# piwell/CS348B-pbrt

Hardware: AMD Instinct MI355X
Metric: volumetric photon-gather throughput (camera samples through PhotonVolumeIntegrator::Li per second) (higher is better)
Workload: dtype f32

## Files before the change

cs348b-pbrt_amd/csrc/pvol_api.hip:

```cpp
#include <hip/hip_runtime.h>
#include <math.h>
#include <stdlib.h>
#include <string.h>
#include <algorithm>
#include <mutex>
#include <new>
#include <vector>

#include "pvol_dev.h"

#include "pvol_host.h"

static bool ok(hipError_t e) { return e == hipSuccess; }

extern "C" {

int pvol_abi_version(void) { return PVOL_ABI_VERSION; }

const char *pvol_strerror(int s) {
    switch (s) {
    case PVOL_OK: return "ok";
    case PVOL_E_INVALID: return "invalid argument";
    case PVOL_E_NO_DEVICE: return "no usable HIP device (this library has no CPU path)";
    case PVOL_E_NO_SCENE: return "no scene set";
// ... 12 lines not shown
}

void pvol_default_params(pvol_params *p) {
    memset(p, 0, sizeof(*p));
    p->step_size = 1.f;
    p->n_used = 250;
    p->max_dist = 0.1f;
    p->n_volume_photons = 0;
    p->shooter_step_size = 0.1f;
    p->max_photon_depth = 5;
    p->n_caustic_photons = 20000;
    p->n_indirect_photons = 10000;
    p->final_gather = 1;
    p->device = 0;
    p->grid_cell_scale = 0.f;
    p->keep_surface_photons = 0;
}

int pvol_create(const pvol_params *params, pvol_ctx **out) {
    if (!params || !out) return PVOL_E_INVALID;
    *out = 0;
    if (params->n_used < 1 || !(params->step_size > 0.f) || !(params->max_dist > 0.f)) return PVOL_E_INVALID;
    if (params->n_used > 576) return PVOL_E_UNSUPPORTED;
    int n = 0;
    if (!ok(hipGetDeviceCount(&n)) || n <= 0 || params->device < 0 || params->device >= n) return PVOL_E_NO_DEVICE;
    if (!ok(hipSetDevice(params->device))) return PVOL_E_NO_DEVICE;
    pvol_ctx *c = new (std::nothrow) pvol_ctx();
    if (!c) return PVOL_E_NO_MEMORY;
    c->params = *params;
    { const char *fs = getenv("PVOL_FORCE_SEQ"); c->forceSeq = fs && fs[0] == '1'; }
    { const char *ng = getenv("PVOL_NO_GROUP"); c->noGroup = ng && ng[0] == '1'; }
    { const char *nl = getenv("PVOL_NO_LITE"); c->noLite = nl && nl[0] == '1'; }
    { const char *nm = getenv("PVOL_NO_MOMENTS"); c->noMoments = nm && nm[0] == '1'; }
    { const char *tg = getenv("PVOL_TILE_GENERAL"); c->tileGeneral = tg && tg[0] == '1'; }
    { const char *gw = getenv("PVOL_GROUP_WAVES"); if (gw) c->groupWavesPerCU = std::max(1, atoi(gw)); }
    { const char *tw = getenv("PVOL_TILE_WAVES"); if (tw) c->tileWaves = std::max(0, atoi(tw)); }
    { const char *fw = getenv("PVOL_FIX_WAVES"); if (fw) c->fixWavesPerCU = std::max(1, atoi(fw)); }
    { const char *lc = getenv("PVOL_LI_COALESCE"); const long v = lc ? atol(lc) : 0; c->coMaxBatch = (v > 1 && v <= PVOL_LI_MAX_BATCH) ? (uint32_t)v : 0u; }
    { hipDeviceProp_t prop; if (ok(hipGetDeviceProperties(&prop, params->device))) c->nCU = prop.multiProcessorCount; }
    if (!c->ds.alloc(1) || !c->dCounters.alloc(1) || !c->dWords.alloc(4) || !c->dsh.alloc(1) ||
        !ok(hipMemset(c->dCounters.get(), 0, sizeof(DevCounters)))) {
        delete c;
        return PVOL_E_NO_DEVICE;
    }
    *out = c;
    return PVOL_OK;
}

void pvol_destroy(pvol_ctx *c) {
    if (!c) return;
    hipSetDevice(c->params.device);
    hipDeviceSynchronize();
    for (auto &p : c->pending) { hipEventDestroy(p.first); hipEventDestroy(p.second); }
    for (auto &p : c->pool) { hipEventDestroy(p.first); hipEventDestroy(p.second); }
    for (auto &p : c->phaseMarks) hipEventDestroy(p.second);
    for (auto &e : c->phasePool) hipEventDestroy(e);
    if (c->groupFilmEv) hipEventDestroy(c->groupFilmEv);
    if (c->groupStageEv) hipEventDestroy(c->groupStageEv);
    pvol_free_li_staging(c);
    delete c;
}

int pvol_get_accel_info(pvol_ctx *c, double *out2) {
    if (!c || !out2) return PVOL_E_INVALID;
    out2[0] = (double)c->hs.nBvhTris; out2[1] = c->bvhBuildMs;
    return PVOL_OK;
// ... 98 lines not shown
        p.specCap = std::min<size_t>(cap, (size_t)1 << 24);
    }
}

void pvol_plan_batch(const PlanIn *in, BatchPlan *out) {
    *out = plan_path(*in);
    if (out->rc == PVOL_OK) plan_size(*in, *out);
}

static float moment_sig_bar(const float *sigA, const float *sigS, double *maxDelta) {
    float lo = INFINITY, hi = -INFINITY;
    for (int b = 0; b < PVOL_NBINS; ++b) { const float t = sigA[b] + sigS[b]; lo = std::min(lo, t); hi = std::max(hi, t); }
    const float bar = (float)(0.5 * ((double)lo + (double)hi));
    *maxDelta = std::max((double)hi - (double)bar, (double)bar - (double)lo);
    return bar;
}
static int moment_terms(const float *sigA, const float *sigS, double pathBound, int maxN) {
    double maxDelta = 0.0;
    const float bar = moment_sig_bar(sigA, sigS, &maxDelta);
    if (!std::isfinite(bar) || !std::isfinite(pathBound) || !(pathBound >= 0.0)) return 0;
    const double x = maxDelta * pathBound;
    double term = exp(x);
    for (int n = 1; n <= maxN; ++n) {
        term *= x / n;
        if (term < ldexp(1.0, -25)) return n;
    }
    return 0;
}
int pvol_moment_gate(const float *sigA, const float *sigS, double pathBound) {
    if (!sigA || !sigS) return 0;
    return moment_terms(sigA, sigS, pathBound, MOM_ORDERS);
}

static double extent_world_diagonal(const DevScene &h) {
    const float *w = h.w2v;
    if (w[12] != 0.f || w[13] != 0.f || w[14] != 0.f || w[15] != 1.f) return INFINITY;
    const double m[3][3] = {{w[0], w[1], w[2]}, {w[4], w[5], w[6]}, {w[8], w[9], w[10]}};
    const double det = m[0][0] * (m[1][1] * m[2][2] - m[1][2] * m[2][1]) - m[0][1] * (m[1][0] * m[2][2] - m[1][2] * m[2][0]) +
                       m[0][2] * (m[1][0] * m[2][1] - m[1][1] * m[2][0]);
    if (!std::isfinite(det) || det == 0.0) return INFINITY;
    double inv[3][3];
    for (int i = 0; i < 3; ++i)
        for (int j = 0; j < 3; ++j) {
            const int a = (j + 1) % 3, b = (j + 2) % 3, c = (i + 1) % 3, d = (i + 2) % 3;
            inv[i][j] = (m[a][c] * m[b][d] - m[a][d] * m[b][c]) / det;
        }
    const double e[3] = {(double)h.extHi[0] - h.extLo[0], (double)h.extHi[1] - h.extLo[1], (double)h.extHi[2] - h.extLo[2]};
    double best = 0.0;
    for (int s = 0; s < 4; ++s) {
        const double v[3] = {e[0], (s & 1) ? -e[1] : e[1], (s & 2) ? -e[2] : e[2]};
        double l2 = 0.0;
        for (int i = 0; i < 3; ++i) { const double u = inv[i][0] * v[0] + inv[i][1] * v[1] + inv[i][2] * v[2]; l2 += u * u; }
        best = std::max(best, sqrt(l2));
    }
    return best * (1.0 + 1e-6);
}

int pvol_moment_scene(DevScene &h, MomentWeights *wts) {
    h.momSigBar = 0.f;
    memset(h.momEmit, 0, sizeof(h.momEmit)); memset(h.momDirect, 0, sizeof(h.momDirect));
    if (wts) memset(wts, 0, sizeof(*wts));
    if (h.volKind != PVOL_VOLUME_HOMOGENEOUS) return 0;
    const double diag = extent_world_diagonal(h);
    const int terms = moment_terms(h.sigA, h.sigS, diag, MOM_ORDERS);
    if (terms < 1 || moment_terms(h.sigA, h.sigS, 2.0 * diag, MOM_ORDERS + 1) < 1) return 0;
    double maxDelta = 0.0;
// ... 205 lines not shown
int pvol_launch_batch(pvol_ctx *c, const BatchArgs &b) {
    PlanIn in = plan_input(c, b);
    BatchPlan p = plan_path(in);
    if (p.rc != PVOL_OK) return p.rc;
    const hipStream_t stream = b.stream;
    std::pair<hipEvent_t, hipEvent_t> ev;
    {
        std::lock_guard<std::mutex> g(c->mu);
        harvest_events(c, false);
        if (!c->pool.empty()) { ev = c->pool.back(); c->pool.pop_back(); }
        else if (!ok(hipEventCreate(&ev.first)) || !ok(hipEventCreate(&ev.second))) return PVOL_E_NO_DEVICE;
    }
    struct EventReturn {
        pvol_ctx *c; std::pair<hipEvent_t, hipEvent_t> ev; bool keep = false;
        ~EventReturn() { if (!keep) { std::lock_guard<std::mutex> g(c->mu); c->pool.push_back(ev); } }
    } evGuard{c, ev};
    if (p.path == PVOL_PATH_SLICED && in.maxRays == 0) {
        std::vector<pvol_stream> hs(b.nStreams);
        if (!ok(hipMemcpyAsync(hs.data(), b.streams, sizeof(pvol_stream) * (size_t)b.nStreams, hipMemcpyDeviceToHost, stream)) ||
            !ok(hipStreamSynchronize(stream))) return PVOL_E_NO_DEVICE;
        for (uint32_t i = 0; i < b.nStreams; ++i) in.maxRays = std::max(in.maxRays, hs[i].n_rays);
    }
    plan_size(in, p);
    int rc = reserve_scratch(c, p, stream);
    if (rc != PVOL_OK) return rc;
    c->lastKernel = p.kernel;
    TileArgs tile;
    if (b.tile) tile = *b.tile;
    LiArgs a = {};
    a.scene = c->ds.get(); a.rays = b.rays; a.streams = b.streams; a.nStreams = b.nStreams; a.nRays = b.nRays; a.outputKind = b.outputKind;
    a.out = b.out; a.draws = b.draws; a.initState = b.initState; a.finalState = b.finalState; a.counters = c->dCounters.get();
    a.transmittanceOnly = b.transOnly; a.chunkCounter = c->dWords.get(); a.needSeq = c->dWords.get() + 1; a.gated = 0;
    a.tauOut = b.tauOut; a.status = b.status; a.grpGuess = in.knobs.groupGuess; a.moments = p.groupForm == GRP_FORM_MOMENTS;
    if (p.groupForm) {
        a.defer = pvol_buf<DeferRec>(c, PVOL_BUF_DEFER); a.deferCount = c->dWords.get() + 2;
        a.deferCap = (uint32_t)std::min<size_t>(c->buf[PVOL_BUF_DEFER].bytes / sizeof(DeferRec), 0xffffffffu);
        if (p.path == PVOL_PATH_SLICED) { a.fxgWiden = in.knobs.fxgWiden; a.fxgAim = in.knobs.fxgAim; }
    }
    if (p.path == PVOL_PATH_PAR) hipMemsetAsync(c->dWords.get(), 0, 3 * sizeof(uint32_t), stream);
    if (p.tile == PVOL_TILE_COUNT) {
        a.sliceK = 0; a.sliceM = 0xffffffc0u; a.state = 0;
        if (p.specCap) rc = spec_pool_reset(c, &tile, p.specCap, stream);
        if (rc == PVOL_OK) rc = run_tile_count(c, b, p, a, &tile);
        if (rc != PVOL_OK) return rc;
    }
    hipEventRecord(ev.first, stream);
    pvol_phase_mark(c, stream, PVOL_PHASE_MARCH);
    rc = p.path == PVOL_PATH_PAR ? run_par(c, b, p, a) : p.path == PVOL_PATH_SLICED ? run_sliced(c, b, p, a, &tile) : run_seq(c, b, p, a);
    if (rc != PVOL_OK) return rc;
    hipEventRecord(ev.second, stream);
    pvol_phase_mark(c, stream, PVOL_PHASE_END);
    std::lock_guard<std::mutex> g(c->mu);
    c->pending.push_back(ev);
    evGuard.keep = true;
    return PVOL_OK;
}

static int check_errors(pvol_ctx *c) {
    DevCounters h;
    if (!ok(hipMemcpy(&h, c->dCounters.get(), sizeof(h), hipMemcpyDeviceToHost))) return PVOL_E_NO_DEVICE;
    if (h.nErrors) {
        unsigned long long zero = 0;
        hipMemcpy(&c->dCounters.get()->nErrors, &zero, sizeof(zero), hipMemcpyHostToDevice);
        return PVOL_E_LIMIT;
    }
    return PVOL_OK;
// ... 164 lines not shown
```

cs348b-pbrt_amd/csrc/pvol_dev.h:

```cpp
#ifndef PVOL_DEV_H
#define PVOL_DEV_H

#include <stdint.h>
#include "../../include/pvol.h"

#define PVOL_MAX_LIGHTS 8
#define PVOL_MAX_TRIS 64
#define PVOL_BVH_MAX_TRIS (1 << 24)
#define PVOL_MAX_SPHERES 8
#define PVOL_MAX_RING 8

#ifdef __HIPCC__
__host__ __device__
#endif
static inline bool is_density_region(int kind) { return kind == PVOL_VOLUME_GRID || kind == PVOL_VOLUME_EXPONENTIAL; }

struct DevLight {
    int32_t kind;
    float pos[3];
    float dir[3];
    float w2l[12];
    float cosTotalWidth, cosFalloffStart;
    float intensity[32];
};

struct DevSphere {
    float o2w[16], w2o[16];
    float radius, zmin, zmax, thetaMin, thetaMax, phiMax;
    int32_t mat, flip;
};

struct DevTri {
    float p1[3], p2[3], p3[3];
};

struct DevSurfMap {
    uint32_t nPhotons;
    int32_t nPaths;
    float gridLo[3];
    float cellSize, invCell;
    int32_t gdim[3];
    const uint32_t *cellStart;
    const float4 *pos4, *alpha4, *wi4;
};
#define SURF_MAP_CAUSTIC 0
#define SURF_MAP_INDIRECT 1
struct DevSurface {
    int32_t enabled, nLookup, maxSpecularDepth;
// ... 154 lines not shown
```

cs348b-pbrt_amd/csrc/pvol_group_dev.h:

```cpp
#define GRP_CH 512
#define GRP_CAP 256
#define GRP_NW (GRP_CAP / 32)
#define GRP_BINS 64
#define GRP_PITCH (GRP_CAP + 4)
#define GRP_WIDEN 1.7f
#define GRP_MINI 8
#ifndef GRP_CORE_MIN
#define GRP_CORE_MIN 8
#endif
#define GRP_TRI_ROWS 8
#define GRP_WPE 3
#define GRP_U_BYTES 4096
#define GRP_PLAN_KMAX 100

struct GroupLds {
    float *pos;
    uint32_t *hist;
    float *miniD;
    float *ubuf;
    unsigned short *order;
    float *cst;
    float *trows;
    float *lint;
};

__device__ float grid_tau_lane(const DevScene &S, V3 o, V3 d, float mint, float maxt, float stepSize, float u) {
    const float length = len(d);
    if (length == 0.f) return 0.f;
    RayD rn;
    rn.o = o; rn.d = vdiv(d, length); rn.mint = mint * length; rn.maxt = maxt * length;
    float t0, t1;
    if (!vol_intersect(S, rn, &t0, &t1)) return 0.f;
    float dsum = 0.f;
    t0 += u * stepSize;
    while (t0 < t1) {
        dsum += region_density(S, xform_point(S.w2v, rn.o + rn.d * t0));
        t0 += stepSize;
    }
    return dsum * stepSize;
}

template <int CAP, bool FINE = false, bool IDX_ONLY = false>
__device__ int stage_bucket_g(const GridView &S, Gather &G, float *bucket, V3 c, float Rs, int lane, unsigned long long &tested) {
    constexpr int GRP_PITCH_ = CAP + 4;
    float *bX = bucket, *bY = bucket + GRP_PITCH_, *bZ = bucket + 2 * GRP_PITCH_, *bI = IDX_ONLY ? bucket : bucket + 3 * GRP_PITCH_;
    const float T = Rs * Rs;
    const GridRows rows = grid_rows<FINE>(S, c, Rs, 0);
    int count = 0;
    for (int rb = 0; rb < rows.nrows; rb += LANES) {
        uint32_t start, rlen;
        grid_row_range<FINE>(S, rows, rb + lane, c, T, &start, &rlen);
        const uint32_t lenS = rlen <= PAINT_ROW ? rlen : 0u;
        uint32_t incl = lenS;
        incl += (uint32_t)__builtin_amdgcn_update_dpp(0, (int)incl, 0x111, 0xf, 0xf, true);
        incl += (uint32_t)__builtin_amdgcn_update_dpp(0, (int)incl, 0x112, 0xf, 0xf, true);
        incl += (uint32_t)__builtin_amdgcn_update_dpp(0, (int)incl, 0x114, 0xf, 0xf, true);
        incl += (uint32_t)__builtin_amdgcn_update_dpp(0, (int)incl, 0x118, 0xf, 0xf, true);
        incl += (uint32_t)__builtin_amdgcn_update_dpp(0, (int)incl, 0x142, 0xa, 0xf, false);
        incl += (uint32_t)__builtin_amdgcn_update_dpp(0, (int)incl, 0x143, 0xc, 0xf, false);
        const uint32_t off = incl - lenS;
        const uint32_t total = (uint32_t)lane_i((int)incl, LANES - 1);
        tested += total;
        uint64_t longRows = __ballot(rlen > PAINT_ROW);
        if (total) {
            __syncthreads();
            for (uint32_t it = 0; it < PAINT_ROW; ++it) {
                if (!wave_any(it < lenS)) break;
                if (it < lenS) G.paint[off + it] = start + it;
            }
            __syncthreads();
        }
        uint32_t segBase = 0u, segLen = total;
        bool painted = true;
        for (;;) {
            for (uint32_t cb = 0; cb < segLen; cb += LANES * NCH) {
                f4 P[NCH];
                uint32_t I[NCH];
                bool on[NCH];
#pragma unroll
                for (int k = 0; k < NCH; ++k) {
                    on[k] = false;
                    I[k] = 0u;
                    P[k] = mk4(0.f);
                    if (cb + k * LANES < segLen) {
                        uint32_t g = cb + k * LANES + lane;
                        on[k] = g < segLen;
                        if (on[k]) {
                            I[k] = painted ? G.paint[g] : segBase + g;
                            P[k] = S.pos4[I[k]];
                        }
                    }
                }
#pragma unroll
                for (int k = 0; k < NCH; ++k) {
                    if (cb + k * LANES >= segLen) continue;
                    float dx = P[k].x - c.x, dyy = P[k].y - c.y, dzz = P[k].z - c.z;
                    float d2 = dx * dx + dyy * dyy + dzz * dzz;
                    bool acc = on[k] && d2 < T;
                    uint64_t m = __ballot(acc);
                    if (m) {
                        const int add = __popcll(m);
                        if (count + add > CAP) return -1;
                        if (acc) {
                            const int at = count + (int)lanes_below(m, lane);
                            if (!IDX_ONLY) { bX[at] = P[k].x; bY[at] = P[k].y; bZ[at] = P[k].z; }
                            bI[at] = __uint_as_float(I[k]);
                        }
                        count += add;
                    }
                }
            }
            if (!longRows) break;
            const int j = __ffsll((unsigned long long)longRows) - 1;
            longRows &= longRows - 1;
            painted = false;
            segBase = (uint32_t)lane_i((int)start, j);
            segLen = (uint32_t)lane_i((int)rlen, j);
            tested += segLen;
        }
    }
    if (IDX_ONLY) { if (lane < 8) bI[count + lane] = 0.f; }
    else if (lane < 4) { bX[count + lane] = 3.0e18f; bY[count + lane] = 3.0e18f; bZ[count + lane] = 3.0e18f; bI[count + lane] = 0.f; }
    __syncthreads();
    return count;
}
__device__ __forceinline__ int stage_bucket(const DevScene &S, Gather &G, float *bucket, V3 c, float Rs, int lane, unsigned long long &tested) {
    const GridView g = volume_grid(S);
    return stage_bucket_g<GRP_CAP>(g, G, bucket, c, Rs, lane, tested);
}

typedef float nf4 __attribute__((ext_vector_type(4)));
typedef float f32x16 __attribute__((ext_vector_type(16)));
#ifndef GRP_PHASE_DIAG
#define GRP_PHASE_DIAG 0
#endif

__device__ __forceinline__ uint32_t wave_or(uint32_t v) {
    v |= (uint32_t)__builtin_amdgcn_update_dpp(0, (int)v, DPP_QUAD_XOR1, 0xf, 0xf, true);
    v |= (uint32_t)__builtin_amdgcn_update_dpp(0, (int)v, DPP_QUAD_XOR2, 0xf, 0xf, true);
    v |= (uint32_t)__builtin_amdgcn_update_dpp(0, (int)v, DPP_ROW_HALF_MIRROR, 0xf, 0xf, true);
    v |= (uint32_t)__builtin_amdgcn_update_dpp(0, (int)v, DPP_ROW_ROR8, 0xf, 0xf, true);
    { auto r = __builtin_amdgcn_permlane16_swap(v, v, false, false); v = r[0] | r[1]; }
    { auto r = __builtin_amdgcn_permlane32_swap(v, v, false, false); v = r[0] | r[1]; }
    return v;
}

template <bool EXACT>
__device__ __forceinline__ uint32_t grp_bin(float d2, float scale, float Tl) {
    uint32_t bin = (uint32_t)fminf(d2 * scale, (float)GRP_BINS);
    if (EXACT) bin = d2 < Tl ? min(bin, (uint32_t)(GRP_BINS - 1)) : (uint32_t)GRP_BINS;
    return bin;
}

typedef float nf2 __attribute__((ext_vector_type(2)));
__device__ __forceinline__ nf2 pk_sub_lo(nf2 a, nf2 pp) {
    nf2 r;
    asm("v_pk_add_f32 %0, %1, %2 op_sel_hi:[1,0] neg_lo:[0,1] neg_hi:[0,1]" : "=v"(r) : "v"(a), "v"(pp));
    return r;
}
__device__ __forceinline__ nf2 pk_sub_hi(nf2 a, nf2 pp) {
    nf2 r;
// ... 303 lines not shown
                        }
                    }
                    const bool black = (fallReg == 0.f) || ((lightBlackMask >> ln) & 1u);
                    if (!black && !(rowsOK ? tri_rows_occluded(L.trows, S.nTris, vis.o, vis.d, vis.mint, vis.maxt) : lane_occluded(S, vis))) {
                        lit = true;
                        V3 dv = xform_vector(S.w2v, vis.d);
                        V3 dvInv = v3(1.f / dv.x, 1.f / dv.y, 1.f / dv.z);
                        exitLen = GRID ? grid_tau_lane(S, vis.o, vis.d, vis.mint, vis.maxt, 4.f * S.stepSize, rec.stepU[2 * j + 1])
                                       : inside_exit_length(S, vis.o, vis.d, pv, dvInv, vis.maxt);
                        ph = phase_hg(-d, -wo, S.g);
                        ++uCount;
                    }
                }
                wc.steps += __popcll(__ballot(act));
                if (STATS) wc.unocc += __popcll(__ballot(lit));
                const float kRem = -1.442695041f * (totalLen - cumLen);
                const float stepD = step * dens;
                const unsigned long long tq1 = (STATS && GRP_PHASE_DIAG == 2) ? stamp() : 0ull;
                if (STATS && GRP_PHASE_DIAG == 2) wc.diag0 += tq1 - tq0;
                f32x16 CA, CB;
                nf4 CM[4];
#pragma unroll
                for (int b = 0; b < 16; ++b) { CA[b] = 0.f; CB[b] = 0.f; }
#pragma unroll
                for (int g = 0; g < 4; ++g) CM[g] = nf4{0.f, 0.f, 0.f, 0.f};
                bool anyFlux = false;
                float rk = 0.f;
                int nFoundLane = k;
                const bool need = inP && S.nPhotons > 0u && useLiiAny;
                bool done = !need;
                if (__ballot(need)) {
                    float guessBase = lastRk;
                    if (j < PREV_N) guessBase = fmaxf(guessBase, prevRk[j]);
                    {
                        const float nbr = wave_max(lastRk);
                        if (!(guessBase > 0.f)) guessBase = nbr > 0.f ? nbr : S.rkEstimate;
                    }
                    float Twant = need ? ((!fixedR && guessBase * A.grpGuess < S.maxDistSq) ? guessBase * A.grpGuess : S.maxDistSq) : 0.f;
                    int lastFail = 0;
                    for (int attempt = 0; attempt < 3; ++attempt) {
                        bool needP = need && !done && Twant > 0.f;
                        if (!__ballot(needP)) break;
                        float Tl = Twant;
                        if (attempt < 2) {
                            const float Tmin = -wave_max(needP ? -Tl : -3.0e38f);
                            needP = needP && !(Tl > 3.f * Tmin);
                        }
                        const float gbl = Tl;
                        bool fullR = !(Tl < S.maxDistSq);
                        float T = needP ? Tl : 0.f;
                        T = wave_max(T);
                        const float big = 3.0e38f;
                        float lx = needP ? p.x : big, ly = needP ? p.y : big, lz = needP ? p.z : big;
                        float hx = needP ? p.x : -big, hy = needP ? p.y : -big, hz = needP ? p.z : -big;
                        lx = -wave_max(-lx); ly = -wave_max(-ly); lz = -wave_max(-lz);
                        hx = wave_max(hx); hy = wave_max(hy); hz = wave_max(hz);
                        V3 c = v3(0.5f * (lx + hx), 0.5f * (ly + hy), 0.5f * (lz + hz));
                        float rho = needP ? len(p - c) : 0.f;
                        rho = wave_max(rho);
                        if (attempt < 2 && rho > 0.3f * sqrtf(T)) {
                            const float ex = hx - lx, ey = hy - ly, ez = hz - lz;
                            const float side = (ex >= ey && ex >= ez) ? p.x - c.x : (ey >= ez ? p.y - c.y : p.z - c.z);
                            needP = needP && !(side > 0.f);
                            T = wave_max(needP ? Tl : 0.f);
                            lx = needP ? p.x : big; ly = needP ? p.y : big; lz = needP ? p.z : big;
                            hx = needP ? p.x : -big; hy = needP ? p.y : -big; hz = needP ? p.z : -big;
                            lx = -wave_max(-lx); ly = -wave_max(-ly); lz = -wave_max(-lz);
                            hx = wave_max(hx); hy = wave_max(hy); hz = wave_max(hz);
                            c = v3(0.5f * (lx + hx), 0.5f * (ly + hy), 0.5f * (lz + hz));
                            rho = wave_max(needP ? len(p - c) : 0.f);
                        }
                        const float Rs = (sqrtf(T) + rho) * 1.0001f + 1e-6f;
                        unsigned long long tst = 0, ts0 = STATS ? stamp() : 0ull;
                        __syncthreads();
                        const int Mb = stage_bucket(S, G, L.pos, c, Rs, lane, tst);
                        if (STATS) { wc.tested += (unsigned long long)max(Mb, 0); wc.cySearch += stamp() - ts0; }
                        if (STATS) wc.diag5 += 1;
                        if (Mb < 0) {
                            if (STATS && !GRP_PHASE_DIAG) wc.diag1 += __popcll(__ballot(needP));
                            if (needP) { Twant = fixedR ? 0.f : 0.4f * Tl; lastFail = 1; }
                            continue;
                        }
                        if (needP) {
                            const float cover = (sqrtf(T) + rho) - len(p - c);
                            Tl = fminf(S.maxDistSq, fmaxf(Tl, fminf(cover * cover, gbl * GRP_WIDEN)));
                            fullR = !(Tl < S.maxDistSq);
                        }
                        const unsigned long long tp1 = STATS ? stamp() : 0ull;
                        const nf2 pxy = {p.x, p.y}, pz_ = {p.z, p.z};
                        const float scale = needP ? (float)GRP_BINS / Tl : 0.f;
                        const bool exact = __ballot(needP && fullR) != 0ull;
#pragma unroll
                        for (int wd = 0; wd <= GRP_BINS / 8; ++wd) histLane[wd * LANES] = 0u;
                        if (exact) grp_pass1<true>(bX, bY, bZ, Mb, pxy, pz_, scale, Tl, histLane);
                        else grp_pass1<false>(bX, bY, bZ, Mb, pxy, pz_, scale, Tl, histLane);
                        const unsigned long long tpa = (STATS && GRP_PHASE_DIAG == 1) ? stamp() : 0ull;
                        if (STATS && GRP_PHASE_DIAG == 1) wc.diag1 += tpa - tp1;
                        int cum = 0, wsel = -1, cumWord = 0;
                        uint32_t selBits = 0u;
#pragma unroll
                        for (int wd = 0; wd < GRP_BINS / 8; ++wd) {
                            const uint32_t w = histLane[wd * LANES];
                            const int t = (int)nib_sum(w);
                            const bool here = wsel < 0 && cum + t >= k;
                            wsel = here ? wd : wsel;
                            selBits = here ? w : selBits;
                            cumWord = here ? cum : cumWord;
                            cum += t;
                        }
                        const int inRange = ((Mb + 3) & ~3) - (int)histLane[(GRP_BINS / 8) * LANES];
                        int bstarI = -1, cumBelow = 0, binCount = 0;
                        {
                            int c2 = cumWord;
#pragma unroll
                            for (int s = 0; s < 8; ++s) {
                                const int cb = (int)((selBits >> (4 * s)) & 15u);
                                const bool here = bstarI < 0 && c2 + cb >= k;
                                bstarI = here ? 8 * wsel + s : bstarI;
                                cumBelow = here ? c2 : cumBelow;
                                binCount = here ? cb : binCount;
                                c2 += cb;
                            }
                        }
                        const bool sane = needP && cum == inRange;
                        bool ok = sane && wsel >= 0 && bstarI >= 0 && binCount <= GRP_MINI;
                        const bool shortSet = sane && fullR && inRange < k;
                        const bool tooFew = needP && !fullR && cum < k;
                        if (STATS && !GRP_PHASE_DIAG && attempt == 0) wc.diag0 += __popcll(__ballot(needP && !ok && !shortSet));
                        if (needP) {
                            Twant = 0.f;
                            lastFail = tooFew ? 2 : 3;
                            if (!tooFew && !ok && !shortSet) Twant = (sane && bstarI >= 0) ? Tl * ((float)(bstarI + 1) * (1.f / GRP_BINS)) * 1.001f : 0.6f * Tl;
                            if (tooFew) {
                                const float grow = cum > 0 ? 1.35f * __builtin_amdgcn_exp2f(0.6666667f * __builtin_amdgcn_logf((float)k / (float)cum)) : 1.0e9f;
                                Twant = fminf(S.maxDistSq, Tl * fmaxf(1.5f, grow));
                            }
                        }
                        const bool planLane = ok || shortSet;
                        const unsigned long long tpb = (STATS && GRP_PHASE_DIAG == 1) ? stamp() : 0ull;
                        if (STATS && GRP_PHASE_DIAG == 1) wc.diag0 += tpb - tpa;
                        if (__ballot(planLane)) {
                            uint32_t mem[GRP_NW], le[GRP_NW];
                            float dmax = 0.f;
                            const uint32_t bstar = shortSet ? (uint32_t)GRP_BINS : (ok ? (uint32_t)bstarI : 0u);
                            float th1, th2;
                            bool thOK = true;
                            if (exact) { th1 = grp_theta<true>(bstar, scale, Tl, &thOK); th2 = grp_theta<true>(bstar + 1u, scale, Tl, &thOK); }
                            else { th1 = grp_theta<false>(bstar, scale, Tl, &thOK); th2 = grp_theta<false>(bstar + 1u, scale, Tl, &thOK); }
                            ok = ok && thOK;
                            __syncthreads();
                            if (exact) grp_pass2<true>(bX, bY, bZ, Mb, pxy, pz_, th1, th2, mem, le, dmax);
                            else grp_pass2<false>(bX, bY, bZ, Mb, pxy, pz_, th1, th2, mem, le, dmax);
                            const unsigned long long tpc = (STATS && GRP_PHASE_DIAG == 1) ? stamp() : 0ull;
                            if (STATS && GRP_PHASE_DIAG == 1) wc.diag3 += tpc - tpb;
                            int nb = 0;
#pragma unroll
                            for (int wd = 0; wd < GRP_NW; ++wd) {
                                if (wd * 32 >= Mb) continue;
                                uint32_t ib = ok ? (le[wd] & ~mem[wd]) : 0u;
                                while (__ballot(ib != 0u)) {
                                    const bool v = ib != 0u;
                                    const int slot = wd * 32 + (v ? __builtin_ctz(ib) : 0);
                                    const float dx = bX[slot] - p.x, dy = bY[slot] - p.y, dz = bZ[slot] - p.z;
                                    const float d2 = dx * dx + dy * dy + dz * dz;
                                    if (v && nb < GRP_MINI) L.miniD[nb * LANES + lane] = d2;
                                    nb += v ? 1 : 0;
                                    ib &= ib - 1u;
                                }
                            }
                            __syncthreads();
                            float sv[GRP_MINI];
#pragma unroll
                            for (int t = 0; t < GRP_MINI; ++t) sv[t] = t < nb ? L.miniD[t * LANES + lane] : INFINITY;
#pragma unroll
                            for (int rnd = 0; rnd < GRP_MINI; ++rnd) {
#pragma unroll
                                for (int t = rnd & 1; t + 1 < GRP_MINI; t += 2) {
                                    const float lo = fminf(sv[t], sv[t + 1]), hi = fmaxf(sv[t], sv[t + 1]);
                                    sv[t] = lo; sv[t + 1] = hi;
                                }
                            }
                            const int m = k - cumBelow;
                            float rkC = sv[0];
#pragma unroll
                            for (int t = 1; t < GRP_MINI; ++t) rkC = (m == t + 1) ? sv[t] : rkC;
                            int nLessIn = 0;
#pragma unroll
                            for (int t = 0; t < GRP_MINI; ++t) nLessIn += (sv[t] < rkC) ? 1 : 0;
                            int quota = m - nLessIn;
                            ok = ok && nb == binCount && rkC < INFINITY;
                            {
                                int t2 = 0;
#pragma unroll
                                for (int wd = 0; wd < GRP_NW; ++wd) {
                                    if (wd * 32 >= Mb) continue;
                                    uint32_t ib = ok ? (le[wd] & ~mem[wd]) : 0u;
                                    while (__ballot(ib != 0u)) {
                                        const bool v = ib != 0u;
                                        const uint32_t bit = v ? (ib & (0u - ib)) : 0u;
                                        const float dv = L.miniD[min(t2, GRP_MINI - 1) * LANES + lane];
                                        const bool tie = v && dv == rkC && quota > 0;
                                        if (tie) --quota;
                                        if (v && (dv < rkC || tie)) mem[wd] |= bit;
                                        t2 += v ? 1 : 0;
                                        ib &= ib - 1u;
                                    }
                                }
                            }
                            if (shortSet) { ok = thOK; rkC = dmax; }
                            const unsigned long long tp3 = STATS ? stamp() : 0ull;
                            if (STATS) wc.cySelect += tp3 - tp1;
                            if (STATS && GRP_PHASE_DIAG == 1) wc.diag4 += tp3 - tpc;
                            const int half = lane >> 5, binL = lane & 31;
                            typedef const __attribute__((address_space(1))) float gfloat;
                            gfloat *alphaF = (gfloat *)(S.alpha4);
                            if (MOMENTS) {
                            const int qtr = lane >> 4, rowL = lane & 15;
                            gfloat *momF = (gfloat *)(S.mom);
                            auto quarters = [](uint32_t v, uint32_t (&w)[4]) {
                                auto h2 = __builtin_amdgcn_permlane32_swap(v, v, false, false);
                                auto lo = __builtin_amdgcn_permlane16_swap(h2[0], h2[0], false, false);
                                auto hi = __builtin_amdgcn_permlane16_swap(h2[1], h2[1], false, false);
                                w[0] = lo[0]; w[1] = lo[1]; w[2] = hi[0]; w[3] = hi[1];
                            };
                            if (GRP_CORE_MIN < GRP_CAP) {
                                const bool anyOk = __ballot(ok) != 0ull;
                                int nCore = 0;
                                uint32_t coreW[GRP_NW];
#pragma unroll
                                for (int wd = 0; wd < GRP_NW; ++wd) {
                                    coreW[wd] = 0u;
                                    if (wd * 32 >= Mb || !anyOk) continue;
                                    coreW[wd] = (uint32_t)__builtin_amdgcn_readfirstlane((int)~wave_or(ok ? ~mem[wd] : 0u));
                                    nCore += __builtin_popcount(coreW[wd]);
                                }
                                if (nCore >= GRP_CORE_MIN) {
                                    uint32_t *clist = reinterpret_cast<uint32_t *>(L.miniD);
                                    int basePos = 0;
#pragma unroll
                                    for (int r2 = 0; r2 < GRP_NW / 2; ++r2) {
                                        if (r2 * 64 >= Mb) continue;
                                        const unsigned long long c64 = (unsigned long long)coreW[2 * r2] | ((unsigned long long)coreW[2 * r2 + 1] << 32);
                                        if ((c64 >> lane) & 1ull) clist[basePos + (int)lanes_below(c64, lane)] = __float_as_uint(bI[r2 * 64 + lane]);
                                        basePos += __popcll(c64);
                                    }
                                    __syncthreads();
                                    float cs = 0.f;
                                    for (int c0 = 0; c0 < nCore; c0 += 32) {
                                        float v[8];
#pragma unroll
                                        for (int q2 = 0; q2 < 8; ++q2) {
                                            const int at = c0 + 4 * q2 + qtr;
                                            const bool on = at < nCore;
                                            const uint32_t idx = clist[on ? at : 0];
                                            const float w = momF[(size_t)idx * MOM_ROW + rowL];
                                            v[q2] = on ? w : 0.f;
                                        }
                                        cs += ((v[0] + v[1]) + (v[2] + v[3])) + ((v[4] + v[5]) + (v[6] + v[7]));
                                    }
                                    { auto r = __builtin_amdgcn_permlane32_swap(__float_as_uint(cs), __float_as_uint(cs), false, false); cs = __uint_as_float(r[0]) + __uint_as_float(r[1]); }
                                    { auto r = __builtin_amdgcn_permlane16_swap(__float_as_uint(cs), __float_as_uint(cs), false, false); cs = __uint_as_float(r[0]) + __uint_as_float(r[1]); }
                                    uint32_t okQ[4];
                                    quarters(ok ? 1u : 0u, okQ);
#pragma unroll
                                    for (int g = 0; g < 4; ++g)
                                        CM[g] = __builtin_amdgcn_mfma_f32_16x16x4f32(cs, qtr ? 0.f : (float)okQ[g], CM[g], 0, 0, 0);
                                    anyFlux = true;
#pragma unroll
                                    for (int wd = 0; wd < GRP_NW; ++wd) mem[wd] &= ~coreW[wd];
                                    __syncthreads();
                                }
                            }
#pragma unroll
                            for (int wd = 0; wd < GRP_NW; ++wd) {
                                if (wd * 32 >= Mb) continue;
                                const uint32_t mine = ok ? mem[wd] : 0u;
                                uint32_t any = (uint32_t)__builtin_amdgcn_readfirstlane((int)(wave_or(mine)));
                                if (!any) continue;
                                anyFlux = true;
                                uint32_t W[4];
                                quarters(mine, W);
                                while (any) {
                                    uint32_t sel[4], wid[4];
                                    float av[4];
                                    bool on[4];
#pragma unroll
// ... 6 lines not shown
                                            bq[u] = more ? __builtin_ctz(any) : (u ? bq[0] : 0);
                                            cnt += more ? 1 : 0;
                                            any &= any - 1u;
                                        }
                                        sel[t] = (uint32_t)(qtr == 0 ? bq[0] : (qtr == 1 ? bq[1] : (qtr == 2 ? bq[2] : bq[3])));
                                        wid[t] = qtr < cnt ? 1u : 0u;
                                        av[t] = 0.f;
                                        if (on[t]) {
                                            const uint32_t idx = __float_as_uint(bI[wd * 32 + sel[t]]);
                                            av[t] = momF[(size_t)idx * MOM_ROW + rowL];
                                        }
                                    }
#pragma unroll
                                    for (int t = 0; t < 4; ++t) {
                                        if (!on[t]) continue;
#pragma unroll
                                        for (int g = 0; g < 4; ++g)
                                            CM[g] = __builtin_amdgcn_mfma_f32_16x16x4f32(av[t], (float)__builtin_amdgcn_ubfe(W[g], sel[t], wid[t]), CM[g], 0, 0, 0);
                                    }
                                }
                            }
                            } else {
                            if (GRP_CORE_MIN < GRP_CAP) {
                                const bool anyOk = __ballot(ok) != 0ull;
                                int nCore = 0;
                                uint32_t coreW[GRP_NW];
#pragma unroll
                                for (int wd = 0; wd < GRP_NW; ++wd) {
                                    coreW[wd] = 0u;
                                    if (wd * 32 >= Mb || !anyOk) continue;
                                    coreW[wd] = (uint32_t)__builtin_amdgcn_readfirstlane((int)~wave_or(ok ? ~mem[wd] : 0u));
                                    nCore += __builtin_popcount(coreW[wd]);
                                }
                                if (nCore >= GRP_CORE_MIN) {
                                    uint32_t *clist = reinterpret_cast<uint32_t *>(L.miniD);
                                    int basePos = 0;
#pragma unroll
                                    for (int r2 = 0; r2 < GRP_NW / 2; ++r2) {
                                        if (r2 * 64 >= Mb) continue;
                                        const unsigned long long c64 = (unsigned long long)coreW[2 * r2] | ((unsigned long long)coreW[2 * r2 + 1] << 32);
                                        if ((c64 >> lane) & 1ull) clist[basePos + (int)lanes_below(c64, lane)] = __float_as_uint(bI[r2 * 64 + lane]);
                                        basePos += __popcll(c64);
                                    }
                                    __syncthreads();
                                    float cs = 0.f;
                                    for (int c0 = 0; c0 < nCore; c0 += 16) {
                                        float v[8];
#pragma unroll
                                        for (int q2 = 0; q2 < 8; ++q2) {
                                            const int at = c0 + 2 * q2 + half;
                                            const bool on = at < nCore;
                                            const uint32_t idx = clist[on ? at : 0];
                                            const float w = alphaF[(size_t)idx * 32 + binL];
                                            v[q2] = on ? w : 0.f;
                                        }
                                        cs += ((v[0] + v[1]) + (v[2] + v[3])) + ((v[4] + v[5]) + (v[6] + v[7]));
                                    }
                                    { auto r = __builtin_amdgcn_permlane32_swap(__float_as_uint(cs), __float_as_uint(cs), false, false); cs = __uint_as_float(r[0]) + __uint_as_float(r[1]); }
                                    const uint32_t okW = ok ? 1u : 0u;
                                    auto ro = __builtin_amdgcn_permlane32_swap(okW, okW, false, false);
                                    const float fA = half ? 0.f : (float)ro[0], fB = half ? 0.f : (float)ro[1];
                                    CA = __builtin_amdgcn_mfma_f32_32x32x2f32(cs, fA, CA, 0, 0, 0);
                                    CB = __builtin_amdgcn_mfma_f32_32x32x2f32(cs, fB, CB, 0, 0, 0);
                                    anyFlux = true;
#pragma unroll
                                    for (int wd = 0; wd < GRP_NW; ++wd) mem[wd] &= ~coreW[wd];
                                    __syncthreads();
                                }
                            }
#pragma unroll
                            for (int wd = 0; wd < GRP_NW; ++wd) {
                                if (wd * 32 >= Mb) continue;
                                const uint32_t mine = ok ? mem[wd] : 0u;
                                auto sw = __builtin_amdgcn_permlane32_swap(mine, mine, false, false);
                                const uint32_t W1 = sw[0], W2 = sw[1];
                                uint32_t any = (uint32_t)__builtin_amdgcn_readfirstlane((int)(wave_or(W1 | W2)));
                                if (!any) continue;
                                anyFlux = true;
                                const int idxW = (int)__float_as_uint(bI[wd * 32 + binL]);
                                while (any) {
                                    int sel[4];
                                    float av[4];
                                    bool on[4], two[4];
#pragma unroll
                                    for (int t = 0; t < 4; ++t) {
                                        on[t] = any != 0u;
                                        const int b0 = on[t] ? __builtin_ctz(any) : 0;
                                        any &= any - 1u;
                                        two[t] = any != 0u;
                                        const int b1 = two[t] ? __builtin_ctz(any) : b0;
                                        any &= any - 1u;
                                        sel[t] = half ? b1 : b0;
                                        av[t] = 0.f;
                                        if (on[t]) {
                                            const uint32_t i0 = (uint32_t)__builtin_amdgcn_readlane(idxW, b0), i1 = (uint32_t)__builtin_amdgcn_readlane(idxW, b1);
                                            av[t] = alphaF[(size_t)(half ? i1 : i0) * 32 + binL];
                                        }
                                    }
#pragma unroll
                                    for (int t = 0; t < 4; ++t) {
                                        if (!on[t]) continue;
                                        const bool live = two[t] || !half;
                                        const float f1 = live ? (float)((W1 >> sel[t]) & 1u) : 0.f, f2 = live ? (float)((W2 >> sel[t]) & 1u) : 0.f;
                                        CA = __builtin_amdgcn_mfma_f32_32x32x2f32(av[t], f1, CA, 0, 0, 0);
                                        CB = __builtin_amdgcn_mfma_f32_32x32x2f32(av[t], f2, CB, 0, 0, 0);
                                    }
                                }
                            }
                            }
                            if (ok) { done = true; rk = rkC; if (shortSet) nFoundLane = inRange; }
                            if (STATS) { wc.kept += (unsigned long long)k * __popcll(__ballot(ok)); wc.cyFlux += stamp() - tp3; }
                        }
                    }
                    const uint64_t todo = __ballot(need && !done);
                    if (todo) {
                        const bool padded = A.fixGroup != 0;
                        const int nfb = padded ? LANES : __popcll(todo);
                        uint32_t base = 0;
                        if (lane == 0) base = atomicAdd(A.deferCount, (uint32_t)nfb);
                        base = (uint32_t)lane_i((int)base, 0);
                        if (padded || (need && !done)) {
                            const uint32_t at = base + (padded ? (uint32_t)lane : lanes_below(todo, lane));
                            if (at < A.deferCap) {
                                DeferRec r;
                                r.ray = (need && !done) ? (uint32_t)ri : 0xffffffffu; r.px = p.x; r.py = p.y; r.pz = p.z; r.kRem = kRem; r.stepD = stepD;
                                r.guess = fixedR ? 0.f : (Twant > 0.f ? Twant * (1.f / PVOL_GUESS_SCALE) : (guessBase > 0.f ? guessBase : 0.f)); r.dens = dens;
                                A.defer[at] = r;
                            } else {
                                atomicOr(A.needSeq, 1u);
                            }
                        }
                        if (STATS && !GRP_PHASE_DIAG) { wc.retries += nfb; wc.diag3 += __popcll(__ballot(need && !done && lastFail == 1)); wc.diag4 += __popcll(__ballot(need && !done && lastFail == 2)); }
                    }
                    const float rkGuess = (need && done) ? (nFoundLane >= k ? rk : S.maxDistSq) : 0.f;
                    {
                        const float sr = wave_sum(rkGuess), sn = (float)__popcll(__ballot(rkGuess > 0.f));
                        if (j < PREV_N && lane == 0 && sn > 0.f) prevRk[j] = sr / sn;
                    }
                    if (need) lastRk = rkGuess;
                }
                const unsigned long long tq2 = (STATS && GRP_PHASE_DIAG == 2) ? stamp() : 0ull;
                if (STATS && GRP_PHASE_DIAG == 2) wc.diag1 += tq2 - tq1;
                float liiScale = 0.f;
// ... 243 lines not shown
```

cs348b-pbrt_amd/csrc/pvol_host.h:

```cpp
#ifndef PVOL_HOST_H
#define PVOL_HOST_H
#include <hip/hip_runtime.h>
#include <atomic>
#include <condition_variable>
#include <deque>
#include <functional>
#include <mutex>
#include <vector>
#include "pvol_dev.h"

#define PVOL_LOCAL __attribute__((visibility("hidden")))

template <class T> struct PVOL_LOCAL DevPtr {
    DevPtr() {}
    DevPtr(DevPtr &&o) : p(o.release()) {}
    DevPtr &operator=(DevPtr &&o) { reset(o.release()); return *this; }
    DevPtr(const DevPtr &) = delete;
    DevPtr &operator=(const DevPtr &) = delete;
    ~DevPtr() { reset(); }
    bool alloc(size_t count) {
        reset();
        if (hipMalloc(&p, sizeof(T) * count) == hipSuccess) return true;
        p = 0; (void)hipGetLastError();
        return false;
// ... 113 lines not shown
    uint32_t n = 0;
    int depth = 0;
    DevPtr<float4> nodes4;
    DevPtr<float> wi;
};

struct pvol_ctx {
    pvol_params params = {};
    bool haveScene = false;
    DevScene hs = {};
    DevPtr<DevScene> ds;
    DevPtr<float> dDensity;
    DevPtr<float4> dBvhNodes, dBvhTris;
    std::vector<int32_t> triMatHost;
    uint32_t nSceneTris = 0;
    DevPtr<float> dTriN;
    double bvhBuildMs = 0.0;
    DevPtr<float> dRawP, dRawWi, dRawAlpha;
    PhotonGrid volMap;
    DevPtr<DevCounters> dCounters;
    DevPtr<uint32_t> dWords;
    int nCU = 256;
    float maxDensity = 1.f;
    bool noLite = false;
    const char *lastKernel = "";
    const char *lastTileKernel = "";
    const char *lastTileForm = "";
    bool tileGeneral = false;
    int fixWavesPerCU = 16;
    int groupWavesPerCU = 12;
    bool noGroup = false;
    bool forceSeq = false;
    bool noMoments = false;
    int momentTerms = 0;
    bool statsOn = false;
    std::vector<std::pair<hipEvent_t, hipEvent_t> > pending;
    std::vector<std::pair<hipEvent_t, hipEvent_t> > pool;
    double timeMs = 0.0;
    uint64_t launches = 0;
    std::mutex mu;
    int tileWaves = 0;
    bool phaseOn = false;
    std::vector<std::pair<int, hipEvent_t> > phaseMarks;
    std::vector<hipEvent_t> phasePool;
    double phaseMs[PVOL_N_PHASES] = {0, 0, 0, 0, 0, 0};
    std::recursive_mutex apiMu;
    DevBuf buf[PVOL_N_BUFS];
    DevShootScene hsh = {};
    DevPtr<DevShootScene> dsh;
    uint64_t shootStats[12] = {};
    struct PVOL_LOCAL SurfStore { DevPtr<float> p, wo, alpha; uint32_t n = 0, nPaths = 0; } surf[3];
    bool surfKept = false;
    DevPtr<float> dRad;
    uint32_t nRad = 0;
    RadianceResult rad;
    GatherMap gather;
    uint64_t fgScratchBound = 0;
    PhotonGrid causticMap;
    PhotonGrid indirectMap;
    bool specOn = false;
    pvol_stream hSegStream = {};
    double exchangeSeconds = 0.0;
    double prepSeconds[2] = {0.0, 0.0};
    std::atomic<uint32_t> coMaxBatch{0};
    uint32_t coMaxWaitUs = 0;
    std::mutex coMu;
// ... 40 lines not shown
    int32_t nLights, volKind; float g; uint32_t nPhotons; int32_t nUsed, candCap, maxSteps, nTris;
    int32_t roulette, distant;
    int32_t forceSeq, noGroup, noLite, statsOn, nCU, groupWavesPerCU, fixWavesPerCU, tileWaves;
    uint32_t nRays, nStreams, maxRays; int32_t hasInit, transOnly, hasTile; uint32_t spp; int32_t specOn, hasTauOut;
    int16_t momentTerms; int8_t outXYZ, noMoments;
    LaunchKnobs knobs;
};
enum { PVOL_PATH_PAR, PVOL_PATH_SLICED, PVOL_PATH_SEQ };
enum { PVOL_TILE_NONE, PVOL_TILE_COUNT, PVOL_TILE_GRID_COUNT, PVOL_TILE_FUSED };
struct BatchPlan {
    int32_t rc, path, tile;
    int32_t groupForm;
    int32_t fixGroup, liteResolve;
    int32_t resolve;
    uint32_t recStride, sliceM, nSlices, nWaves, gWaves, fixWaves; int32_t tileWavesPerTask;
    uint64_t recBytes, stateBytes, deferWant, specCap, ldsSeq, ldsPar, ldsResolve, ldsGroup, ldsTile;
    const char *kernel;
};
static_assert(sizeof(PlanIn) == 152 && sizeof(BatchPlan) == 136, "tests/test_launch_plan.py mirrors both");
extern "C" size_t pvol_rec_stride(int maxSteps, bool grid);
extern "C" BatchPlan plan_path(const PlanIn &in);
extern "C" void plan_size(const PlanIn &in, BatchPlan &p);
#define GRP_FORM_MOMENTS 3
struct TilePlainIn {
    int32_t tile;
    int32_t volKind, nLights, light0Kind;
    int32_t hasBvh, nSpheres, nTris;
    int32_t surfOn, specLink;
    int32_t tileGeneral;
};
static_assert(sizeof(TilePlainIn) == 40, "tests/test_tile_plain_gate.py mirrors it");
extern "C" int pvol_tile_plain_gate(const TilePlainIn *in);
extern "C" int pvol_moment_gate(const float *sigA, const float *sigS, double pathBound);
struct MomentWeights { float w[12][32]; };
extern "C" int pvol_moment_scene(DevScene &h, MomentWeights *w);
extern "C" hipError_t pvol_fill_moments(const MomentWeights *w, const float4 *alpha4, float *mom, uint32_t n, hipStream_t stream);

extern "C" {
void pvol_phase_mark(pvol_ctx *c, hipStream_t stream, int id);
int pvol_finish_map(pvol_ctx *c, uint32_t n, const float *hostPositions);
void pvol_free_photons(pvol_ctx *c);
void pvol_free_surface_stores(pvol_ctx *c);
void pvol_free_caustic_map(pvol_ctx *c);
int pvol_push_scene(pvol_ctx *c);
int pvol_li_lone(pvol_ctx *c, const pvol_ray *ray, uint32_t *mt, int32_t *mti, float *Lv, float *T);
int pvol_li_coalesced(pvol_ctx *c, const pvol_ray *ray, uint32_t *mt, int32_t *mti, float *Lv, float *T);
void pvol_free_li_staging(pvol_ctx *c);
int pvol_order_after_pending(pvol_ctx *c, hipStream_t stream);
void *pvol_rccl_symbol(const char *name);
void pvol_plan_batch(const PlanIn *in, BatchPlan *out);
int pvol_gather_tree_build(const float *p, uint32_t n, void *nodes, int32_t *depth);
struct GatherCheck {
    const pvol_photon_array *indirect;
    const float *p; uint32_t count; float maxDist;
    const void *outIndex, *outD2, *outFound, *outRounds;
    const float *frames, *wo, *uBsdf, *uPhoton; int32_t nSamples; float cosGatherAngle; const void *outBsdf, *outPhoton;
};
int pvol_check_gather(int what, int haveCtx, int haveState, uint32_t storeN, const GatherCheck *args, int hostPointers);
struct FinalGatherCheck {
    const float *p, *frames, *wo, *kd, *rayEps; uint32_t count; float maxDist; int32_t nSamples; float cosGatherAngle;
    const float *uBsdf, *uPhoton; const void *L, *draws;
};
int pvol_check_final_gather(int haveCtx, const FinalGatherCheck *args, int haveScene, int volKind, int haveGather, int haveRad, uint32_t radN);
uint32_t pvol_final_gather_slice(int32_t nSamples, uint64_t bound);
int pvol_final_gather_set_scratch_bound(pvol_ctx *c, uint64_t bytes);
size_t pvol_shoot_merge_replay(const uint32_t *cfg, const uint32_t *tables, uint32_t nTables, uint64_t *out, size_t cap);
// ... 69 lines not shown
```

cs348b-pbrt_amd/csrc/pvol_liargs.h:

```cpp
#ifndef PVOL_LIARGS_H
#define PVOL_LIARGS_H
#include "pvol_dev.h"
struct LiArgs {
    const DevScene *scene;
    const pvol_ray *rays;
    pvol_stream *streams;
    uint32_t nStreams;
    uint32_t nRays;
    int outputKind;
    float *out;
    uint32_t *draws;
    const uint32_t *initState;
    uint32_t *finalState;
    DevCounters *counters;
    int transmittanceOnly;
    uint32_t *chunkCounter;
    uint32_t *needSeq;
    int gated;
    unsigned char *records;
    uint32_t recStride, sliceM, sliceK;
    uint32_t *state;
    float grpGuess;
    int liteResolve;
    DeferRec *defer;
    uint32_t *deferCount;
    uint32_t deferCap;
    TauRec *tauOut;
    int32_t fixGroup;
    float fxgWiden, fxgAim;
    int32_t *status;
    int32_t moments;
};
#endif
```

Before: 148.6.

## Pre-classify photons inside a guaranteed-core radius during group bucket staging

```diff
diff --git a/cs348b-pbrt_amd/csrc/pvol_api.hip b/cs348b-pbrt_amd/csrc/pvol_api.hip
--- a/cs348b-pbrt_amd/csrc/pvol_api.hip
+++ b/cs348b-pbrt_amd/csrc/pvol_api.hip
@@ -68,6 +68,7 @@
     { const char *ng = getenv("PVOL_NO_GROUP"); c->noGroup = ng && ng[0] == '1'; }
     { const char *nl = getenv("PVOL_NO_LITE"); c->noLite = nl && nl[0] == '1'; }
     { const char *nm = getenv("PVOL_NO_MOMENTS"); c->noMoments = nm && nm[0] == '1'; }
+    c->groupPrecore = pvol_precore_kappa(getenv("PVOL_GROUP_PRECORE"));
     { const char *tg = getenv("PVOL_TILE_GENERAL"); c->tileGeneral = tg && tg[0] == '1'; }
     { const char *gw = getenv("PVOL_GROUP_WAVES"); if (gw) c->groupWavesPerCU = std::max(1, atoi(gw)); }
     { const char *tw = getenv("PVOL_TILE_WAVES"); if (tw) c->tileWaves = std::max(0, atoi(tw)); }
@@ -232,6 +233,15 @@
     return moment_terms(sigA, sigS, pathBound, MOM_ORDERS);
 }
 
+float pvol_precore_bound(float theta, float rho) { return precore_bound(theta, rho); }
+float pvol_precore_kappa(const char *env) {
+    if (!env || !env[0]) return PVOL_PRECORE_DEFAULT;
+    char *end = 0;
+    const float v = strtof(env, &end);
+    if (end == env || !(v >= 0.f)) return PVOL_PRECORE_DEFAULT;
+    return std::min(v, 1.f);
+}
+
 static double extent_world_diagonal(const DevScene &h) {
     const float *w = h.w2v;
     if (w[12] != 0.f || w[13] != 0.f || w[14] != 0.f || w[15] != 1.f) return INFINITY;
@@ -503,6 +513,7 @@
     a.out = b.out; a.draws = b.draws; a.initState = b.initState; a.finalState = b.finalState; a.counters = c->dCounters.get();
     a.transmittanceOnly = b.transOnly; a.chunkCounter = c->dWords.get(); a.needSeq = c->dWords.get() + 1; a.gated = 0;
     a.tauOut = b.tauOut; a.status = b.status; a.grpGuess = in.knobs.groupGuess; a.moments = p.groupForm == GRP_FORM_MOMENTS;
+    a.grpPrecore = c->groupPrecore;
     if (p.groupForm) {
         a.defer = pvol_buf<DeferRec>(c, PVOL_BUF_DEFER); a.deferCount = c->dWords.get() + 2;
         a.deferCap = (uint32_t)std::min<size_t>(c->buf[PVOL_BUF_DEFER].bytes / sizeof(DeferRec), 0xffffffffu);
diff --git a/cs348b-pbrt_amd/csrc/pvol_dev.h b/cs348b-pbrt_amd/csrc/pvol_dev.h
--- a/cs348b-pbrt_amd/csrc/pvol_dev.h
+++ b/cs348b-pbrt_amd/csrc/pvol_dev.h
@@ -1,6 +1,7 @@
 #ifndef PVOL_DEV_H
 #define PVOL_DEV_H
 
+#include <math.h>
 #include <stdint.h>
 #include "../../include/pvol.h"
 
@@ -14,6 +15,17 @@
 __host__ __device__
 #endif
 static inline bool is_density_region(int kind) { return kind == PVOL_VOLUME_GRID || kind == PVOL_VOLUME_EXPONENTIAL; }
+
+#ifdef __HIPCC__
+__host__ __device__
+#endif
+static inline float precore_bound(float theta, float rho) {
+    if (!(theta > 0.f) || !(rho >= 0.f)) return 0.f;
+    const float s = sqrtf(theta);
+    if (!(s > rho)) return 0.f;
+    const float r = (s - 1e-6f) / 1.0001f - rho;
+    return r > 0.f ? r * r : 0.f;
+}
 
 struct DevLight {
     int32_t kind;
diff --git a/cs348b-pbrt_amd/csrc/pvol_group_dev.h b/cs348b-pbrt_amd/csrc/pvol_group_dev.h
--- a/cs348b-pbrt_amd/csrc/pvol_group_dev.h
+++ b/cs348b-pbrt_amd/csrc/pvol_group_dev.h
@@ -40,13 +40,16 @@
     return dsum * stepSize;
 }
 
-template <int CAP, bool FINE = false, bool IDX_ONLY = false>
-__device__ int stage_bucket_g(const GridView &S, Gather &G, float *bucket, V3 c, float Rs, int lane, unsigned long long &tested) {
+template <int CAP, bool FINE = false, bool IDX_ONLY = false, bool PRE = false>
+__device__ int stage_bucket_g(const GridView &S, Gather &G, float *bucket, V3 c, float Rs, int lane, unsigned long long &tested,
+                              float dPre = 0.f, int *nPreOut = nullptr) {
+    static_assert(!(PRE && IDX_ONLY), "the settled class lives in the index component of the SoA bucket");
     constexpr int GRP_PITCH_ = CAP + 4;
     float *bX = bucket, *bY = bucket + GRP_PITCH_, *bZ = bucket + 2 * GRP_PITCH_, *bI = IDX_ONLY ? bucket : bucket + 3 * GRP_PITCH_;
     const float T = Rs * Rs;
     const GridRows rows = grid_rows<FINE>(S, c, Rs, 0);
-    int count = 0;
+    int count = 0, nPre = 0;
+    if (PRE) *nPreOut = 0;
     for (int rb = 0; rb < rows.nrows; rb += LANES) {
         uint32_t start, rlen;
         grid_row_range<FINE>(S, rows, rb + lane, c, T, &start, &rlen);
@@ -100,13 +103,18 @@
                     uint64_t m = __ballot(acc);
                     if (m) {
                         const int add = __popcll(m);
-                        if (count + add > CAP) return -1;
-                        if (acc) {
+                        if (count + nPre + add > CAP) return -1;
+                        const bool pre = PRE && acc && d2 < dPre;
+                        const uint64_t mp = PRE ? __ballot(pre) : 0ull;
+                        m &= ~mp;
+                        if (acc && !pre) {
                             const int at = count + (int)lanes_below(m, lane);
                             if (!IDX_ONLY) { bX[at] = P[k].x; bY[at] = P[k].y; bZ[at] = P[k].z; }
                             bI[at] = __uint_as_float(I[k]);
                         }
-                        count += add;
+                        if (PRE && pre) bI[GRP_PITCH_ - 1 - nPre - (int)lanes_below(mp, lane)] = __uint_as_float(I[k]);
+                        count += __popcll(m);
+                        if (PRE) nPre += __popcll(mp);
                     }
                 }
             }
@@ -121,12 +129,14 @@
     }
     if (IDX_ONLY) { if (lane < 8) bI[count + lane] = 0.f; }
     else if (lane < 4) { bX[count + lane] = 3.0e18f; bY[count + lane] = 3.0e18f; bZ[count + lane] = 3.0e18f; bI[count + lane] = 0.f; }
+    if (PRE) *nPreOut = nPre;
     __syncthreads();
     return count;
 }
-__device__ __forceinline__ int stage_bucket(const DevScene &S, Gather &G, float *bucket, V3 c, float Rs, int lane, unsigned long long &tested) {
+__device__ __forceinline__ int stage_bucket(const DevScene &S, Gather &G, float *bucket, V3 c, float Rs, int lane, unsigned long long &tested,
+                                            float dPre, int *nPre) {
     const GridView g = volume_grid(S);
-    return stage_bucket_g<GRP_CAP>(g, G, bucket, c, Rs, lane, tested);
+    return stage_bucket_g<GRP_CAP, false, false, true>(g, G, bucket, c, Rs, lane, tested, dPre, nPre);
 }
 
 typedef float nf4 __attribute__((ext_vector_type(4)));
@@ -496,6 +506,7 @@
                 if (__ballot(need)) {
                     float guessBase = lastRk;
                     if (j < PREV_N) guessBase = fmaxf(guessBase, prevRk[j]);
+                    const bool measured = guessBase > 0.f;
                     {
                         const float nbr = wave_max(lastRk);
                         if (!(guessBase > 0.f)) guessBase = nbr > 0.f ? nbr : S.rkEstimate;
@@ -535,14 +546,26 @@
                             rho = wave_max(needP ? len(p - c) : 0.f);
                         }
                         const float Rs = (sqrtf(T) + rho) * 1.0001f + 1e-6f;
+                        float theta = 0.f;
+                        if (GRP_CORE_MIN < GRP_CAP && attempt == 0 && !fixedR && A.grpPrecore > 0.f && __ballot(needP) &&
+                            !__ballot(needP && (!measured || !(Tl * GRP_WIDEN < S.maxDistSq))))
+                            theta = A.grpPrecore * -wave_max(needP ? -guessBase : -3.0e38f);
+                        int nPre = 0;
                         unsigned long long tst = 0, ts0 = STATS ? stamp() : 0ull;
                         __syncthreads();
-                        const int Mb = stage_bucket(S, G, L.pos, c, Rs, lane, tst);
+                        const int Mb = stage_bucket(S, G, L.pos, c, Rs, lane, tst, precore_bound(theta, rho), &nPre);
                         if (STATS) { wc.tested += (unsigned long long)max(Mb, 0); wc.cySearch += stamp() - ts0; }
                         if (STATS) wc.diag5 += 1;
                         if (Mb < 0) {
                             if (STATS && !GRP_PHASE_DIAG) wc.diag1 += __popcll(__ballot(needP));
                             if (needP) { Twant = fixedR ? 0.f : 0.4f * Tl; lastFail = 1; }
+                            continue;
+                        }
+                        if (nPre == 0) theta = 0.f;
+                        const int kq = k - nPre;
+                        if (kq < 1) {
+                            if (STATS && !GRP_PHASE_DIAG) wc.diag0 += __popcll(__ballot(needP));
+                            if (needP) lastFail = 3;
                             continue;
                         }
                         if (needP) {
@@ -566,7 +589,7 @@
                         for (int wd = 0; wd < GRP_BINS / 8; ++wd) {
                             const uint32_t w = histLane[wd * LANES];
                             const int t = (int)nib_sum(w);
-                            const bool here = wsel < 0 && cum + t >= k;
+                            const bool here = wsel < 0 && cum + t >= kq;
                             wsel = here ? wd : wsel;
                             selBits = here ? w : selBits;
                             cumWord = here ? cum : cumWord;
@@ -579,7 +602,7 @@
 #pragma unroll
                             for (int s = 0; s < 8; ++s) {
                                 const int cb = (int)((selBits >> (4 * s)) & 15u);
-                                const bool here = bstarI < 0 && c2 + cb >= k;
+                                const bool here = bstarI < 0 && c2 + cb >= kq;
                                 bstarI = here ? 8 * wsel + s : bstarI;
                                 cumBelow = here ? c2 : cumBelow;
                                 binCount = here ? cb : binCount;
@@ -588,15 +611,15 @@
                         }
                         const bool sane = needP && cum == inRange;
                         bool ok = sane && wsel >= 0 && bstarI >= 0 && binCount <= GRP_MINI;
-                        const bool shortSet = sane && fullR && inRange < k;
-                        const bool tooFew = needP && !fullR && cum < k;
+                        const bool shortSet = sane && fullR && inRange + nPre < k;
+                        const bool tooFew = needP && !fullR && cum + nPre < k;
                         if (STATS && !GRP_PHASE_DIAG && attempt == 0) wc.diag0 += __popcll(__ballot(needP && !ok && !shortSet));
                         if (needP) {
                             Twant = 0.f;
                             lastFail = tooFew ? 2 : 3;
                             if (!tooFew && !ok && !shortSet) Twant = (sane && bstarI >= 0) ? Tl * ((float)(bstarI + 1) * (1.f / GRP_BINS)) * 1.001f : 0.6f * Tl;
                             if (tooFew) {
-                                const float grow = cum > 0 ? 1.35f * __builtin_amdgcn_exp2f(0.6666667f * __builtin_amdgcn_logf((float)k / (float)cum)) : 1.0e9f;
+                                const float grow = cum + nPre > 0 ? 1.35f * __builtin_amdgcn_exp2f(0.6666667f * __builtin_amdgcn_logf((float)k / (float)(cum + nPre))) : 1.0e9f;
                                 Twant = fminf(S.maxDistSq, Tl * fmaxf(1.5f, grow));
                             }
                         }
@@ -644,7 +667,7 @@
                                     sv[t] = lo; sv[t + 1] = hi;
                                 }
                             }
-                            const int m = k - cumBelow;
+                            const int m = kq - cumBelow;
                             float rkC = sv[0];
 #pragma unroll
                             for (int t = 1; t < GRP_MINI; ++t) rkC = (m == t + 1) ? sv[t] : rkC;
@@ -653,6 +676,11 @@
                             for (int t = 0; t < GRP_MINI; ++t) nLessIn += (sv[t] < rkC) ? 1 : 0;
                             int quota = m - nLessIn;
                             ok = ok && nb == binCount && rkC < INFINITY;
+                            {
+                                const bool unverified = ok && !(rkC >= theta);
+                                if (unverified) { ok = false; Twant = Tl; }
+                                if (STATS && !GRP_PHASE_DIAG && theta > 0.f) wc.diag0 += __popcll(__ballot(unverified));
+                            }
                             {
                                 int t2 = 0;
 #pragma unroll
@@ -698,7 +726,7 @@
                                     coreW[wd] = (uint32_t)__builtin_amdgcn_readfirstlane((int)~wave_or(ok ? ~mem[wd] : 0u));
                                     nCore += __builtin_popcount(coreW[wd]);
                                 }
-                                if (nCore >= GRP_CORE_MIN) {
+                                if (anyOk && (nPre > 0 || nCore >= GRP_CORE_MIN)) {
                                     uint32_t *clist = reinterpret_cast<uint32_t *>(L.miniD);
                                     int basePos = 0;
 #pragma unroll
@@ -708,14 +736,16 @@
                                         if ((c64 >> lane) & 1ull) clist[basePos + (int)lanes_below(c64, lane)] = __float_as_uint(bI[r2 * 64 + lane]);
                                         basePos += __popcll(c64);
                                     }
+                                    for (int i = lane; i < nPre; i += LANES) clist[nCore + i] = __float_as_uint(bI[GRP_PITCH - 1 - i]);
+                                    const int nSum = nCore + nPre;
                                     __syncthreads();
                                     float cs = 0.f;
-                                    for (int c0 = 0; c0 < nCore; c0 += 32) {
+                                    for (int c0 = 0; c0 < nSum; c0 += 32) {
                                         float v[8];
 #pragma unroll
                                         for (int q2 = 0; q2 < 8; ++q2) {
                                             const int at = c0 + 4 * q2 + qtr;
-                                            const bool on = at < nCore;
+                                            const bool on = at < nSum;
                                             const uint32_t idx = clist[on ? at : 0];
                                             const float w = momF[(size_t)idx * MOM_ROW + rowL];
                                             v[q2] = on ? w : 0.f;
@@ -788,7 +818,7 @@
                                     coreW[wd] = (uint32_t)__builtin_amdgcn_readfirstlane((int)~wave_or(ok ? ~mem[wd] : 0u));
                                     nCore += __builtin_popcount(coreW[wd]);
                                 }
-                                if (nCore >= GRP_CORE_MIN) {
+                                if (anyOk && (nPre > 0 || nCore >= GRP_CORE_MIN)) {
                                     uint32_t *clist = reinterpret_cast<uint32_t *>(L.miniD);
                                     int basePos = 0;
 #pragma unroll
@@ -798,14 +828,16 @@
                                         if ((c64 >> lane) & 1ull) clist[basePos + (int)lanes_below(c64, lane)] = __float_as_uint(bI[r2 * 64 + lane]);
                                         basePos += __popcll(c64);
                                     }
+                                    for (int i = lane; i < nPre; i += LANES) clist[nCore + i] = __float_as_uint(bI[GRP_PITCH - 1 - i]);
+                                    const int nSum = nCore + nPre;
                                     __syncthreads();
                                     float cs = 0.f;
-                                    for (int c0 = 0; c0 < nCore; c0 += 16) {
+                                    for (int c0 = 0; c0 < nSum; c0 += 16) {
                                         float v[8];
 #pragma unroll
                                         for (int q2 = 0; q2 < 8; ++q2) {
                                             const int at = c0 + 2 * q2 + half;
-                                            const bool on = at < nCore;
+                                            const bool on = at < nSum;
                                             const uint32_t idx = clist[on ? at : 0];
                                             const float w = alphaF[(size_t)idx * 32 + binL];
                                             v[q2] = on ? w : 0.f;
@@ -864,7 +896,7 @@
                                 }
                             }
                             }
-                            if (ok) { done = true; rk = rkC; if (shortSet) nFoundLane = inRange; }
+                            if (ok) { done = true; rk = rkC; if (shortSet) nFoundLane = inRange + nPre; }
                             if (STATS) { wc.kept += (unsigned long long)k * __popcll(__ballot(ok)); wc.cyFlux += stamp() - tp3; }
                         }
                     }
diff --git a/cs348b-pbrt_amd/csrc/pvol_host.h b/cs348b-pbrt_amd/csrc/pvol_host.h
--- a/cs348b-pbrt_amd/csrc/pvol_host.h
+++ b/cs348b-pbrt_amd/csrc/pvol_host.h
@@ -169,6 +169,7 @@
     bool noGroup = false;
     bool forceSeq = false;
     bool noMoments = false;
+    float groupPrecore = 0.f;
     int momentTerms = 0;
     bool statsOn = false;
     std::vector<std::pair<hipEvent_t, hipEvent_t> > pending;
@@ -275,6 +276,9 @@
 static_assert(sizeof(TilePlainIn) == 40, "tests/test_tile_plain_gate.py mirrors it");
 extern "C" int pvol_tile_plain_gate(const TilePlainIn *in);
 extern "C" int pvol_moment_gate(const float *sigA, const float *sigS, double pathBound);
+#define PVOL_PRECORE_DEFAULT 0.7f
+extern "C" float pvol_precore_bound(float theta, float rho);
+extern "C" float pvol_precore_kappa(const char *env);
 struct MomentWeights { float w[12][32]; };
 extern "C" int pvol_moment_scene(DevScene &h, MomentWeights *w);
 extern "C" hipError_t pvol_fill_moments(const MomentWeights *w, const float4 *alpha4, float *mom, uint32_t n, hipStream_t stream);
diff --git a/cs348b-pbrt_amd/csrc/pvol_liargs.h b/cs348b-pbrt_amd/csrc/pvol_liargs.h
--- a/cs348b-pbrt_amd/csrc/pvol_liargs.h
+++ b/cs348b-pbrt_amd/csrc/pvol_liargs.h
@@ -30,5 +30,6 @@
     float fxgWiden, fxgAim;
     int32_t *status;
     int32_t moments;
+    float grpPrecore;
 };
 #endif
```

Measured after the change: 157.9, median of 6. 6.2% higher.
